# AlexeyAB/yolo2_light

Measured on NVIDIA H100. Metric: images/sec, higher is better.
Workload: dtype bf16

## Files before the change

### yolo2_light_b200/api.py

```python
from __future__ import annotations

import ctypes as C
import os
from typing import List, Optional

import numpy as np

_HERE = os.path.dirname(os.path.abspath(__file__))
LIB_PATH = os.environ.get("YB_LIB") or os.path.join(_HERE, "libyolo2_light_b200.so")

YB_CONVOLUTIONAL, YB_MAXPOOL, YB_SOFTMAX, YB_ROUTE, YB_SHORTCUT = 0, 3, 4, 8, 13
YB_REGION, YB_YOLO, YB_UPSAMPLE, YB_REORG, YB_BLANK = 21, 22, 23, 24, 25
YB_LOGISTIC, YB_RELU, YB_LINEAR, YB_LEAKY = 0, 1, 3, 7
YB_PREC_BF16_TC, YB_PREC_FP32 = 0, 1
YB_QUANT_NONE, YB_QUANT_CPU, YB_QUANT_GPU = 0, 1, 2
LAYER_NAMES = {0: "CONVOLUTIONAL", 3: "MAXPOOL", 4: "SOFTMAX", 8: "ROUTE", 13: "SHORTCUT", 21: "REGION", 22: "YOLO",
               23: "UPSAMPLE", 24: "REORG", 25: "BLANK"}


class YbError(RuntimeError):
    pass


class LayerDesc(C.Structure):
# ... 107 lines not shown
    return L


EXPORTED_SYMBOLS = [
    "yb_set_abort_on_error", "yb_last_error", "yb_version", "yb_parse_network_cfg", "yb_load_weights_upto",
    "yb_fuse_conv_batchnorm", "yb_calculate_binary_weights", "yb_quantinization_and_get_multipliers",
    "yb_network_from_layers", "yb_free_network", "yb_network_num_layers", "yb_network_dims", "yb_network_layer",
    "yb_network_layer_outputs", "yb_network_input_calibration", "yb_set_batch_network", "yb_network_set_device",
    "yb_network_set_precision", "yb_network_set_option", "yb_network_get_info", "yb_network_tc_plan", "yb_network_detect", "yb_network_calibrate", "yb_entropy_calibration",
    "yb_network_input_histogram", "yb_map_evaluate", "yb_network_predict", "yb_network_predict_quantized",
    "yb_network_predict_cudnn_quantized",
    "yb_network_predict_image_u8", "yb_network_fetch_input", "yb_network_submit", "yb_network_collect", "yb_network_layer_output", "yb_network_forward_device", "yb_network_sync_outputs", "yb_network_fetch_layer",
    "yb_network_fetch_counts", "yb_forward_convolutional_layer", "yb_network_weight_arena",
    "yb_network_last_launches", "yb_network_profile", "yb_op_kind_name", "yb_network_op_kernels", "yb_get_network_boxes", "yb_alloc_pinned",
    "yb_free_pinned", "yb_network_submit_u8", "yb_network_collect_detections", "yb_network_set_devices",
    "yb_network_predict_batch", "yb_network_batch_output", "yb_network_replication", "yb_network_predict_frames_u8",
    "yb_network_detect_frames", "yb_network_submit_frames_u8", "yb_network_predict_device_frames",
    "yb_network_submit_device_frames", "yb_network_set_letterbox",
]


TC_PLAN_FIELDS = ("kernel", "kind", "TW", "TH", "BN", "BK", "nt", "bstat", "stages", "sps", "grid", "num_work", "tma_epi",
                  "jshift", "out_ldc")
TC_PLAN_KERNELS = ("k_conv_tc", "k_conv_tc_reg", "k_stem_tc", "k_stem_s2_tc")
TC_PLAN_KINDS = ("bf16", "s8", "xnor", "tf32", "s8_gpu")


def _check(ok: bool):
    if not ok:
        raise YbError(lib().yb_last_error().decode(errors="replace"))


def _np(ptr, count, dtype):
    if not ptr or count <= 0:
        return None
    return np.ctypeslib.as_array(ptr, shape=(count,)).view(dtype)


class Network:

    def __init__(self, handle: int):
        self._h = C.c_void_p(handle)
        self._refresh()

    def _refresh(self):
        d = (C.c_int * 8)()
        lib().yb_network_dims(self._h, d)
# ... 509 lines not shown
```

### yolo2_light_b200/csrc/yb_conv_tc.cu

```cuda
#include <cuda.h>
#include <cuda_bf16.h>
#include <cuda_runtime.h>

#include <algorithm>
#include <climits>
#include <cstdlib>
#include <cstring>
#include <memory>
#include <string>
#include <type_traits>
#include <vector>

#include "yb_conv_tc.cuh"
#include "yb_cuda.h"

namespace yb {

namespace {

constexpr int TC_BM = 128;
constexpr int TC_EPI_WARPS = 8;
constexpr int TC_THREADS = 32 * TC_EPI_WARPS + 32;
constexpr int TC_PRODUCER_WARP = TC_EPI_WARPS;
constexpr int TC_ACC_BAR = 3;
// ... 24 lines not shown
    int yolo_per;
    int PR, row_off;
    int OH, OW, OHp, OWp;
    int size, cblocks, kblocks;
    int BK, BN;
    int stride2;
    int xoff, yoff;
    int stages;
    uint32_t stage_bytes, a_bytes, b_bytes;
    int bstat;
    uint32_t bstat_bytes;
    int tma_epi;
    uint32_t stg_bytes;
    int acc_pitch;
    int pool_fmt, jshift;
    float pool_mult;
    signed char *pool_out; long pool_ldc; int pool_Hp, pool_Wp;
    int sps;
    TcSmem sm;
    uint32_t desc_hi;
    char *out; long out_ldc; int n;
    const char *res;
    const float *bias; int act, act2;
    unsigned long long *stats;
    int dbg;
};

__device__ __forceinline__ uint32_t smem_u32(const void *p) { return (uint32_t)__cvta_generic_to_shared(p); }

__device__ __forceinline__ bool elect_one() {
    uint32_t pred = 0;
    asm volatile(
        "{\n\t.reg .b32 rx;\n\t.reg .pred px;\n\telect.sync rx|px, %1;\n\t@px mov.s32 %0, 1;\n\t}"
        : "+r"(pred) : "r"(0xffffffffu));
    return pred != 0;
}

__device__ __forceinline__ void mbar_init(uint32_t bar, uint32_t count) {
    asm volatile("mbarrier.init.shared::cta.b64 [%0], %1;" ::"r"(bar), "r"(count));
}
__device__ __forceinline__ void mbar_arrive_expect_tx(uint32_t bar, uint32_t bytes) {
    asm volatile("mbarrier.arrive.expect_tx.shared::cta.b64 _, [%0], %1;" ::"r"(bar), "r"(bytes) : "memory");
}
__device__ __forceinline__ void mbar_arrive(uint32_t bar) {
    asm volatile("mbarrier.arrive.shared::cta.b64 _, [%0];" ::"r"(bar) : "memory");
}
// ... 10 lines not shown
    while (!mbar_try_wait(bar, parity))
        if (clock64() - t0 > 4000000000LL) __trap();
}

__device__ __forceinline__ void tma_load_3d(uint32_t dst, const CUtensorMap *tm, uint32_t bar, int c0, int c1, int c2) {
    asm volatile(
        "cp.async.bulk.tensor.3d.shared::cluster.global.tile.mbarrier::complete_tx::bytes [%0], [%1, {%3, %4, %5}], [%2];"
        ::"r"(dst), "l"(tm), "r"(bar), "r"(c0), "r"(c1), "r"(c2) : "memory");
}
__device__ __forceinline__ uint64_t l2_policy_evict_first() {
    uint64_t pol;
    asm volatile("createpolicy.fractional.L2::evict_first.b64 %0, 1.0;" : "=l"(pol));
    return pol;
}
__device__ __forceinline__ void tma_load_3d_hint(uint32_t dst, const CUtensorMap *tm, uint32_t bar, int c0, int c1, int c2, uint64_t pol) {
    asm volatile(
        "cp.async.bulk.tensor.3d.shared::cluster.global.tile.mbarrier::complete_tx::bytes.L2::cache_hint [%0], [%1, {%3, %4, %5}], [%2], %6;"
        ::"r"(dst), "l"(tm), "r"(bar), "r"(c0), "r"(c1), "r"(c2), "l"(pol) : "memory");
}
__device__ __forceinline__ void tma_load_2d(uint32_t dst, const CUtensorMap *tm, uint32_t bar, int c0, int c1) {
    asm volatile(
        "cp.async.bulk.tensor.2d.shared::cluster.global.tile.mbarrier::complete_tx::bytes [%0], [%1, {%3, %4}], [%2];"
        ::"r"(dst), "l"(tm), "r"(bar), "r"(c0), "r"(c1) : "memory");
}
__device__ __forceinline__ void tma_load_5d(uint32_t dst, const CUtensorMap *tm, uint32_t bar, int c0, int c1, int c2,
                                            int c3, int c4) {
    asm volatile(
        "cp.async.bulk.tensor.5d.shared::cluster.global.tile.mbarrier::complete_tx::bytes [%0], [%1, {%3, %4, %5, %6, %7}], [%2];"
        ::"r"(dst), "l"(tm), "r"(bar), "r"(c0), "r"(c1), "r"(c2), "r"(c3), "r"(c4) : "memory");
}

__device__ __forceinline__ void tma_store_3d(const CUtensorMap *tm, uint32_t src, int c0, int c1, int c2) {
    asm volatile("cp.async.bulk.tensor.3d.global.shared::cta.bulk_group [%0, {%2, %3, %4}], [%1];"
                 ::"l"(tm), "r"(src), "r"(c0), "r"(c1), "r"(c2) : "memory");
}
__device__ __forceinline__ void tma_store_commit() { asm volatile("cp.async.bulk.commit_group;" ::: "memory"); }
__device__ __forceinline__ void tma_store_wait_read0() { asm volatile("cp.async.bulk.wait_group.read 0;" ::: "memory"); }
__device__ __forceinline__ void tma_store_wait_all() { asm volatile("cp.async.bulk.wait_group 0;" ::: "memory"); }
__device__ __forceinline__ void named_bar_sync(int id, int nthreads) {
    asm volatile("bar.sync %0, %1;" ::"r"(id), "r"(nthreads) : "memory");
}
__device__ __forceinline__ void prefetch_tmap(const CUtensorMap *tm) { asm volatile("prefetch.tensormap [%0];" ::"l"(tm) : "memory"); }
__device__ __forceinline__ void fence_mbar_init() { asm volatile("fence.mbarrier_init.release.cluster;" ::: "memory"); }
__device__ __forceinline__ void pdl_wait_and_launch() {
    asm volatile("griddepcontrol.wait;" ::: "memory");
    asm volatile("griddepcontrol.launch_dependents;" ::: "memory");
// ... 893 lines not shown
                const unsigned long long dst = optr[px];
                if (dst)
                    *reinterpret_cast<uint4 *>(dst + (unsigned long long)(part * 16)) =
                        *reinterpret_cast<const uint4 *>(a_tile + px * 64 + ((part ^ ((px >> 1) & 3)) << 4));
            }
        } else if (ok) {
#pragma unroll
            for (int g = 0; g < 4; ++g) {
                if (g * 8 >= p.nf) break;
                float r[8];
#pragma unroll
                for (int j = 0; j < 8; ++j) {
                    const float a = __uint_as_float(acc[g * 8 + j]) + bias_s[g * 8 + j];
                    r[j] = (p.act == ACT_LEAKY) ? fmaxf(a, 0.1f * a) : a;
                }
                reinterpret_cast<uint4 *>(orow)[g] = make_uint4(pack_bf16x2(r[0], r[1]), pack_bf16x2(r[2], r[3]),
                                                                pack_bf16x2(r[4], r[5]), pack_bf16x2(r[6], r[7]));
            }
        }
        __syncthreads();
    }
}

constexpr int S2_TW = 16, S2_TH = 8;
constexpr int S2_RW = 2 * S2_TW + 1, S2_RH = 2 * S2_TH + 1;
constexpr int S2_ROWS = 640;
constexpr uint32_t S2_B1 = 0;
constexpr uint32_t S2_BS = 9u * 4096u;
constexpr uint32_t S2_U = S2_BS + 2048u;
constexpr uint32_t S2_SETS_KX = 17u * 1024u;
constexpr uint32_t S2_STG = (uint32_t)S2_ROWS * 64u;
constexpr uint32_t S2_MISC = S2_U + S2_STG + 2u * 8192u;
constexpr int S2_PH = S2_RH + 2, S2_PW = S2_RW + 2, S2_PP = 36;
constexpr size_t S2_SMEM = 1024 + S2_MISC + 4 * (32 + 64 + 256) + 4 * 3 * S2_PH * S2_PP;
static_assert(S2_STG + 2u * 8192u >= 3u * S2_SETS_KX, "sets must fit the shared region");

template <bool U8>
__global__ void __launch_bounds__(256, 2) k_stem_s2_tc(StemTcP p) {
    extern __shared__ uint8_t smem_raw[];
    uint8_t *sm = smem_raw + ((1024u - (smem_u32(smem_raw) & 1023u)) & 1023u);
    const uint32_t base = smem_u32(sm), U = base + S2_U;
    float *bias0_s = reinterpret_cast<float *>(sm + S2_MISC), *bias1_s = bias0_s + 32, *lut = bias1_s + 64, *patch = lut + 256;
    const int t = threadIdx.x, lane = t & 31;
    const int warp = __shfl_sync(0xffffffffu, t >> 5, 0), wg = warp >> 2;
    if constexpr (U8) lut[t] = (float)((double)(float)t / 255.0);
    if (t < 32) bias0_s[t] = p.bias[t];
// ... 91 lines not shown
                Wg<TC_BF16, 32>::mma(ds[c], wg_desc(U + (uint32_t)(5 * wg + c) * 4096u + 32u * k, hi), wg_desc(base + S2_BS + 32u * k, hi), (uint32_t)k);
        wg_commit();
        wg_wait<0>();
#pragma unroll
        for (int c = 0; c < 5; ++c) wg_fence_operand(ds[c]);
        __syncthreads();

        {
#pragma unroll
            for (int c = 0; c < 5; ++c)
#pragma unroll
                for (int h = 0; h < 2; ++h) {
                    const int i = 64 * (5 * wg + c) + rl + 8 * h;
                    if (i >= S2_RW * S2_RH) continue;
                    const int sy = i / S2_RW, sx = i - sy * S2_RW, y = gy0 + sy, x = gx0 + sx;
                    const bool in_img = y >= 0 && y < p.H && x >= 0 && x < p.W;
                    uint32_t v[4];
#pragma unroll
                    for (int j = 0; j < 4; ++j) {
                        float a = ds[c][4 * j + 2 * h] + bias0_s[8 * j + cq], b = ds[c][4 * j + 2 * h + 1] + bias0_s[8 * j + cq + 1];
                        if (leaky0) { a = fmaxf(a, 0.1f * a); b = fmaxf(b, 0.1f * b); }
                        v[j] = in_img ? pack_bf16x2(a, b) : 0u;
                    }
                    const uint32_t set = U + ((sy & 1) ? 9u * 1024u : 0u) + (uint32_t)(sy >> 1) * 1024u + 2u * (uint32_t)cq;
                    auto put = [&](int kx, int ox) {
                        const uint32_t row = set + (uint32_t)kx * S2_SETS_KX + (uint32_t)ox * 64u;
#pragma unroll
                        for (int j = 0; j < 4; ++j)
                            asm volatile("st.shared.b32 [%0], %1;" ::"r"(row + ((uint32_t)(j ^ ((ox >> 1) & 3)) << 4)), "r"(v[j]));
                    };
                    const bool odd = sx & 1, last = sx == 2 * S2_TW;
                    put(odd ? 1 : last ? 2 : 0, last ? (sx >> 1) - 1 : sx >> 1);
                    if (!odd && !last && sx >= 2) put(2, (sx >> 1) - 1);
                }
        }
        asm volatile("fence.proxy.async.shared::cta;" ::: "memory");
        __syncthreads();

        if (tile + (int)gridDim.x < p.ntiles) load_patch(tile + gridDim.x, pv);

        float d[32];
#pragma unroll
        for (int i = 0; i < 32; ++i) d[i] = 0.f;
        wg_fence_operand(d);
        wg_fence();
#pragma unroll
        for (int r = 0; r < 9; ++r) {
            const int ky = r / 3, kx = r % 3;
            const uint32_t a = U + (uint32_t)kx * S2_SETS_KX + ((ky & 1) ? 9u * 1024u : 0u) + (uint32_t)(ky >> 1) * 1024u + (uint32_t)wg * 4096u;
            const uint32_t b = base + S2_B1 + (uint32_t)r * 4096u;
#pragma unroll
            for (int k = 0; k < 2; ++k)
                Wg<TC_BF16, 64>::mma(d, wg_desc(a + 32u * k, hi), wg_desc(b + 32u * k, hi), (r > 0 || k > 0) ? 1u : 0u);
        }
        wg_commit();
        wg_wait<0>();
        wg_fence_operand(d);
        __syncthreads();

        const uint32_t stg = U + S2_STG + (uint32_t)wg * 8192u;
        float b1[16];
#pragma unroll
        for (int j = 0; j < 8; ++j) { b1[2 * j] = bias1_s[8 * j + cq]; b1[2 * j + 1] = bias1_s[8 * j + cq + 1]; }
#pragma unroll
        for (int h = 0; h < 2; ++h) {
            const int q = rl + 8 * h;
#pragma unroll
            for (int j = 0; j < 8; ++j) {
                float a = d[4 * j + 2 * h] + b1[2 * j], b = d[4 * j + 2 * h + 1] + b1[2 * j + 1];
                if (leaky1) { a = fmaxf(a, 0.1f * a); b = fmaxf(b, 0.1f * b); }
                asm volatile("st.shared.b32 [%0], %1;" ::"r"(stg + (uint32_t)q * 128u + ((uint32_t)(j ^ (q & 7)) << 4) + 2u * (uint32_t)cq),
                             "r"(pack_bf16x2(a, b)) : "memory");
            }
        }
        if (wg == 0) named_bar_sync(1, 128);
        else named_bar_sync(2, 128);
#pragma unroll
        for (int k = 0; k < 4; ++k) {
            const int idx = (t & 127) + 128 * k, q = idx >> 3, ch = idx & 7;
            const int oy = oy0 + 4 * wg + (q >> 4), ox = ox0 + (q & 15);
            if (oy < p.OH && ox < p.OW) {
                uint4 o;
                asm volatile("ld.shared.v4.b32 {%0, %1, %2, %3}, [%4];" : "=r"(o.x), "=r"(o.y), "=r"(o.z), "=r"(o.w)
                             : "r"(stg + (uint32_t)q * 128u + ((uint32_t)(ch ^ (q & 7)) << 4)) : "memory");
                *reinterpret_cast<uint4 *>(p.out + ((size_t)(n * p.OHp + oy + 1) * p.OWp + ox + 1) * (size_t)p.out_ldc * 2 + ch * 16) = o;
            }
        }
    }
}

typedef CUresult (*EncodeTiledFn)(CUtensorMap *, CUtensorMapDataType, cuuint32_t, void *, const cuuint64_t *,
                                  const cuuint64_t *, const cuuint32_t *, const cuuint32_t *, CUtensorMapInterleave,
                                  CUtensorMapSwizzle, CUtensorMapL2promotion, CUtensorMapFloatOOBfill);

EncodeTiledFn encode_fn() {
    static EncodeTiledFn fn = nullptr;
    if (!fn) {
        void *p = nullptr;
        cudaDriverEntryPointQueryResult q;
        if (cudaGetDriverEntryPoint("cuTensorMapEncodeTiled", &p, cudaEnableDefault, &q) != cudaSuccess || !p)
            fatal_throw("cuTensorMapEncodeTiled not available from the driver");
        fn = reinterpret_cast<EncodeTiledFn>(p);
    }
    return fn;
}

}

using TcKernel = void (*)(CUtensorMap, CUtensorMap, CUtensorMap, CUtensorMap, CUtensorMap, TcParams);

struct TcPlan {
    CUtensorMap tmA, tmB, tmO, tmO1, tmR;
    TcParams p;
    TcKernel kernel;
    bool reg;
    int grid;
    size_t smem;
    char desc[96];
    DevBuf<unsigned long long> stats;
};

namespace {

int sm_count() {
    int dev = 0, sms = 132;
    cudaGetDevice(&dev);
    cudaDeviceGetAttribute(&sms, cudaDevAttrMultiProcessorCount, dev);
    return sms;
}

bool is_integer(int kind) { return kind == TC_S8 || kind == TC_S8_GPU || kind == TC_XNOR; }
int elem_size(int kind) { return kind == TC_TF32 ? 4 : is_integer(kind) ? 1 : 2; }
int operand_channels(const TcConv &c) { return is_integer(c.kind) ? c.in.ldc : c.l->c; }

bool geometry_ok(const Layer &l) {
    if (l.stride == 1) return (l.size == 3 && l.pad == 1) || (l.size == 1 && l.pad == 0);
    return l.stride == 2 && l.size == 3 && l.pad == 1 && l.h % 2 == 0 && l.w % 2 == 0;
}
// ... 229 lines not shown
    plan_tiles(p, c, reg, sms);
    plan_epilogue(p, c, reg);
    plan_ring(p, reg);
    plan->smem = tc_smem_layout(p, reg);
    p.dbg = c.sw.dbg;
    snprintf(plan->desc, sizeof(plan->desc), "%dx%dx%d -> n%d k%d s%d%s", l.c, l.h, l.w, l.n, l.size, l.stride, reg ? " reg" : "");
    encode_maps(*plan, c, reg);
    plan->grid = std::min(p.num_work, grid_cap(sms, c.sw.grid));
    const bool st = c.sw.stats;
    plan->reg = reg;
    if (reg) plan->kernel = st ? k_conv_tc_reg<true> : k_conv_tc_reg<false>;
    else if (is_integer(c.kind)) plan->kernel = st ? k_conv_tc<true, 2> : k_conv_tc<false, 2>;
    else plan->kernel = st ? k_conv_tc<true, 0> : k_conv_tc<false, 0>;
    if (cudaFuncSetAttribute((const void *)plan->kernel, cudaFuncAttributeMaxDynamicSharedMemorySize, 227 * 1024) != cudaSuccess)
        fatal_throw("cudaFuncSetAttribute(k_conv_tc) failed");
    if (st) {
        plan->stats.ensure(TC_NSTATS * (size_t)plan->grid);
        p.stats = plan->stats.get();
        cudaMemset(p.stats, 0, sizeof(unsigned long long) * TC_NSTATS * plan->grid);
    }
    return plan;
}

struct StemPlan { StemTcP p; int grid; bool s2; };
int tc_stem_supported(const Layer &l, const TV &out) {
    return l.c == 3 && l.size == 3 && l.stride == 1 && l.pad == 1 && (l.n == 16 || l.n == 32) &&
           (l.activation == YB_LEAKY || l.activation == YB_LINEAR) && out.base && out.ldc % 8 == 0 &&
           (reinterpret_cast<uintptr_t>(out.base) & 15) == 0;
}
StemPlanPtr tc_stem_make_plan(const Layer &l, const TV &out, const void *d_w, const float *d_bias) {
    StemPlanPtr sp(new StemPlan());
    StemTcP &p = sp->p;
    p.out = out.base; p.out_ldc = out.ldc; p.w = reinterpret_cast<const __nv_bfloat16 *>(d_w); p.bias = d_bias;
    p.N = out.N; p.H = l.h; p.W = l.w; p.OHp = out.Hp; p.OWp = out.Wp; p.nf = l.n; p.act = l.activation;
    p.npix = (long)out.N * l.h * l.w;
    if (p.npix >= (1L << 31) - 256) fatal_throw("stem plan: more than 2^31 pixels per batch");
    p.ntiles = (int)((p.npix + 127) / 128);
    sp->grid = std::min(p.ntiles, sm_count() * 8);
    return sp;
}
int tc_stem_s2_supported(const Layer &l0, const Layer &l1, const TV &out1) {
    return l0.n == 32 && l1.c == 32 && l1.n == 64 && l1.size == 3 && l1.stride == 2 && l1.pad == 1 && l1.h == l0.h && l1.w == l0.w &&
           l0.h % 2 == 0 && l0.w % 2 == 0 && (l1.activation == YB_LEAKY || l1.activation == YB_LINEAR) && out1.base && out1.P == 1 &&
           out1.H == l0.h / 2 && out1.W == l0.w / 2 && out1.ldc % 8 == 0 && (reinterpret_cast<uintptr_t>(out1.base) & 15) == 0;
}
StemPlanPtr tc_stem_s2_make_plan(const Layer &l0, const Layer &l1, const TV &out1, const void *d_w, const float *d_bias,
// ... 20 lines not shown
void tc_stem_launch(const StemPlan &sp, const float *d_in_nchw, cudaStream_t s) {
    StemTcP p = sp.p;
    p.in = d_in_nchw;
    if (sp.s2) k_stem_s2_tc<false><<<sp.grid, 256, S2_SMEM, s>>>(p);
    else k_stem_tc<false><<<sp.grid, 128, 0, s>>>(p);
}
void tc_stem_launch_u8(const StemPlan &sp, const unsigned char *d_in_hwc, cudaStream_t s) {
    StemTcP p = sp.p;
    p.in8 = d_in_hwc;
    if (sp.s2) k_stem_s2_tc<true><<<sp.grid, 256, S2_SMEM, s>>>(p);
    else k_stem_tc<true><<<sp.grid, 128, 0, s>>>(p);
}

namespace {
int copy_fields(const int (&f)[TC_PLAN_NFIELDS], int *fields, int n) {
    const int k = std::max(0, std::min(n, (int)TC_PLAN_NFIELDS));
    for (int i = 0; i < k; ++i) fields[i] = f[i];
    return k;
}
}

int tc_plan_fields(const TcPlan &plan, int *fields, int n) {
    const TcParams &p = plan.p;
    const int f[TC_PLAN_NFIELDS] = {plan.reg ? TC_PLAN_CONV_REG : TC_PLAN_CONV, p.kind, p.TW, p.TH, p.BN, p.BK,
                                    p.nt, p.bstat, p.stages, p.sps, plan.grid, p.num_work, p.tma_epi, p.jshift,
                                    p.out ? (int)p.out_ldc : 0};
    return copy_fields(f, fields, n);
}

int tc_stem_plan_fields(const StemPlan &sp, int *fields, int n) {
    const int f[TC_PLAN_NFIELDS] = {sp.s2 ? TC_PLAN_STEM_S2 : TC_PLAN_STEM, TC_BF16, sp.s2 ? S2_TW : -1, sp.s2 ? S2_TH : -1,
                                    sp.s2 ? 64 : -1, -1, -1, -1, -1, -1, sp.grid, sp.p.ntiles, -1, -1, (int)sp.p.out_ldc};
    return copy_fields(f, fields, n);
}

void tc_launch(const TcPlan &P, cudaStream_t s) {
    cudaLaunchConfig_t cfg{};
    cfg.gridDim = dim3((unsigned)P.grid); cfg.blockDim = dim3((unsigned)(P.reg ? TCR_THREADS : TC_THREADS));
    cfg.dynamicSmemBytes = P.smem; cfg.stream = s;
    cudaLaunchAttribute attr[1];
    attr[0].id = cudaLaunchAttributeProgrammaticStreamSerialization;
    attr[0].val.programmaticStreamSerializationAllowed = 1;
    cfg.attrs = attr; cfg.numAttrs = 1;
    cudaLaunchKernelEx(&cfg, P.kernel, P.tmA, P.tmB, P.tmO, P.tmO1, P.tmR, P.p);
}

void TcPlanDelete::operator()(TcPlan *plan) const {
    if (plan->p.stats) {
        std::vector<unsigned long long> h(TC_NSTATS * (size_t)plan->grid);
        cudaDeviceSynchronize();
        cudaMemcpy(h.data(), plan->p.stats, h.size() * sizeof(unsigned long long), cudaMemcpyDeviceToHost);
        double m[TC_NSTATS] = {0};
        for (int b = 0; b < plan->grid; ++b) for (int k = 0; k < TC_NSTATS; ++k) m[k] += (double)h[TC_NSTATS * b + k] / plan->grid;
        fprintf(stderr, "TCSTATS %-28s tiles/cta %.1f kb %d sps %d BN %d | producer: wait_empty %.0f tma_issue %.0f total %.0f | ",
                plan->desc, (double)plan->p.num_work / plan->grid, plan->p.kblocks, plan->p.sps, plan->p.BN,
                m[STAT_PROD_WAIT_EMPTY], m[STAT_PROD_TMA_ISSUE], m[STAT_PROD_TOTAL]);
        if (plan->reg)
            fprintf(stderr, "consumers: wait_full %.0f wait_ready %.0f (first item %.0f) total %.0f | store: wait_full %.0f wait_read %.0f\n",
                    m[STAT_CONS_WAIT_FULL], m[STAT_CONS_WAIT_READY], m[STAT_CONS_FIRST_READY], m[STAT_CONS_TOTAL],
                    m[STAT_STORE_WAIT_FULL], m[STAT_STORE_WAIT_READ]);
        else fprintf(stderr, "consumers: wait_full %.0f total %.0f\n", m[STAT_CONS_WAIT_FULL], m[STAT_CONS_TOTAL]);
// ... 7 lines not shown
```

### yolo2_light_b200/csrc/yb_conv_tc.cuh

```cuda
#pragma once
#include <cuda_runtime.h>

#include <memory>

#include "yb_device.cuh"
#include "yb_model.h"

namespace yb {

struct TcSwitches {
    int bn = 0;
    int grid = 0;
    bool no_bstat = false;
    bool stats = false;
    int dbg = 0;
};

struct TcConv {
    TcKind kind = TC_BF16;
    const Layer *l = nullptr;
    TV in{};
    TV out{};
    bool out_bf16 = false;
    TV res{};
// ... 4 lines not shown
    float alpha1 = 0.f;
    const float *mean = nullptr;
    int *acc_out = nullptr;
    float *yolo_out = nullptr;
    int yolo_classes = 0;
    SideFmt pool_fmt = SIDE_NONE;
    float pool_mult = 0.f;
    TV pool_next{};
    TcSwitches sw{};
};

struct TcPlan;
struct StemPlan;
struct TcPlanDelete {
    void operator()(TcPlan *plan) const;
    void operator()(StemPlan *plan) const;
};
using TcPlanPtr = std::unique_ptr<TcPlan, TcPlanDelete>;
using StemPlanPtr = std::unique_ptr<StemPlan, TcPlanDelete>;

int tc_conv_supported(const TcConv &c);
TcPlanPtr tc_make_plan(const TcConv &c);
void tc_launch(const TcPlan &plan, cudaStream_t s);

int tc_stem_supported(const Layer &l, const TV &out);
StemPlanPtr tc_stem_make_plan(const Layer &l, const TV &out, const void *d_w_32x32_bf16, const float *d_bias);
int tc_stem_s2_supported(const Layer &l0, const Layer &l1, const TV &out1);
StemPlanPtr tc_stem_s2_make_plan(const Layer &l0, const Layer &l1, const TV &out1, const void *d_w_32x32_bf16,
                                 const float *d_bias, const void *d_w1_bf16, const float *d_bias1, int max_grid);
void tc_stem_launch(const StemPlan &plan, const float *d_in_nchw, cudaStream_t s);
void tc_stem_launch_u8(const StemPlan &plan, const unsigned char *d_in_hwc, cudaStream_t s);

enum { TC_PLAN_CONV = 0, TC_PLAN_CONV_REG = 1, TC_PLAN_STEM = 2, TC_PLAN_STEM_S2 = 3, TC_PLAN_NFIELDS = 15 };
int tc_plan_fields(const TcPlan &plan, int *fields, int n);
int tc_stem_plan_fields(const StemPlan &plan, int *fields, int n);

}
```

### yolo2_light_b200/csrc/yb_engine.cu

```cuda
#include "yb_engine.h"

#include <cuda_bf16.h>
#include <cuda_runtime.h>
#include <dlfcn.h>

#include <algorithm>
#include <cmath>
#include <cstdlib>
#include <cstring>

#include "yb_conv_tc.cuh"
#include "yb_cuda.h"
#include "yb_kernels.cuh"
#include "yb_detect.cuh"

namespace yb {

const char *op_kind_name(int k) {
    static const char *names[] = {"input", "conv_simt", "conv_tc", "binarize", "conv_xnor", "quantize",
                                  "conv_int8", "maxpool", "upsample", "shortcut", "route_copy", "reorg",
                                  "yolo", "region", "conv_tc_i8", "conv_tc_tf32"};
    return (k >= 0 && k < 16) ? names[k] : "?";
}

// ... 1 lines not shown
static inline size_t dt_size(int dt) { return dt == DT_F32 ? 4 : dt == DT_BF16 ? 2 : dt == DT_S8 ? 1 : 4; }
#define BY_DT(k, dt) ((dt) == DT_F32 ? k<float> : k<__nv_bfloat16>)

struct Op {
    int kind;
    int layer;
    std::function<void(const float *, cudaStream_t)> launch;
    std::function<void(const unsigned char *, cudaStream_t)> launch_u8;
    const void *kernel = nullptr;
};

struct ConvWeights {
    size_t w_f32 = (size_t)-1, w_bf16 = (size_t)-1, w_s8 = (size_t)-1, w_bits = (size_t)-1;
    size_t w_f32km = (size_t)-1;
    size_t bias = (size_t)-1, mean = (size_t)-1;
    int ldw = 0;
    int ldn = 0;
    int cpad = 0;
};

struct Switches {
    bool no_graph, no_nccl, no_tc, no_tf32, no_stem, no_stem_tc, no_stem_u8, no_stem_pool_fuse, no_stem_s2_fuse,
         no_conv_pool_fuse, no_pool_fuse, no_yolo_fuse;
    bool no_fuse;
    bool xnor_tc;
    int xnor_tc_minc;
    TcSwitches tc;
    static Switches read() {
        auto set = [](const char *name) { return getenv(name) != nullptr; };
        auto num = [](const char *name) { const char *v = getenv(name); return v ? atoi(v) : 0; };
        const char *xtc = getenv("YB_XNOR_TC"), *minc = getenv("YB_XNOR_TC_MINC"), *nf = getenv("YB_NO_FUSE");
        return Switches{set("YB_NO_GRAPH"), set("YB_NO_NCCL"), set("YB_NO_TC"), set("YB_NO_TF32"), set("YB_NO_STEM"),
                        set("YB_NO_STEM_TC"), set("YB_NO_STEM_U8"), set("YB_NO_STEM_POOL_FUSE"), set("YB_NO_STEM_S2_FUSE"),
                        set("YB_NO_CONV_POOL_FUSE"), set("YB_NO_POOL_FUSE"), set("YB_NO_YOLO_FUSE"),
                        nf && nf[0] == '1', !(xtc && xtc[0] == '0'), minc ? atoi(minc) : 16,
                        TcSwitches{set("YB_TC_BN") ? std::max(num("YB_TC_BN"), 1) : 0, num("YB_TC_GRID"), set("YB_TC_NO_BSTAT"),
                                   set("YB_TC_STATS"), num("YB_TC_DBG")}};
    }
};

struct Engine {
    EngineOptions opt;
    Switches sw{};
    int batch = 0;
    int act_dt = DT_F32;
    Stream stream;
    DevBuf<char> act_arena, w_arena;
    DevBuf<float> d_input;
    std::vector<TV> out_tv;
    std::vector<int> out_dt;
    struct Final { DevBuf<float> d; PinnedBuf<float> h; };
    std::vector<Final> finals;
    std::vector<DevBuf<int32_t>> counts;
    std::vector<Op> ops;
    TV in0{};
    int in0_dt = DT_F32;
    GraphExec graph_exec;
// ... 64 lines not shown
            if (l.type == YB_SHORTCUT) cons[l.index].push_back(i);
        }
    }
    return cons;
}

template <typename T> struct same_type { using type = T; };


enum FirstOp { FIRST_NHWC, FIRST_STEM_SIMT, FIRST_STEM_TC, FIRST_STEM_S2, FIRST_STEM_POOL };
enum ConvPath { CP_NONE, CP_TC, CP_TF32, CP_SIMT, CP_XNOR_FALLBACK, CP_XNOR_TC, CP_XNOR_SMALLK, CP_XNOR_GENERAL, CP_I8_TC, CP_I8_SIMT };

struct LayerPlan {
    int variant = 0;
    int path = CP_NONE;
    int fused_into = -1;
    bool fused_sc = false;
    bool yolo_fused = false;
    SideFmt pool = SIDE_NONE;
    bool pool_in_conv = false;
    bool pool_to_side = false;
    bool prefilled = false;
    bool in_first_op = false;
    int out_dt = DT_F32;
    SideFmt side = SIDE_NONE;
    int side_ld = 0;
    bool has_out = false;
    bool materialised = false;
    int owner = -1, coff = 0;
    int ldc = 0;
};

static char *const kLayoutBase = reinterpret_cast<char *>(uintptr_t(1) << 40);

template <typename F>
static void for_each_weight(const Layer &l, F &&put) {
    const int taps = l.size * l.size;
    for (int f = 0; f < l.n; ++f)
        for (int c = 0; c < l.c; ++c)
            for (int t = 0; t < taps; ++t) put(f, c, t, ((size_t)f * l.c + c) * taps + t);
}

template <int NF>
static StemW<NF> stem_weights(const Layer &l0) {
    StemW<NF> w{};
    for_each_weight(l0, [&](int f, int c, int t, size_t k) { w.w[(t * 3 + c) * NF + f] = l0.weights[k]; });
// ... 303 lines not shown
    }

    void plan_fusions() {
        for (int i = 0; i < nl; ++i) {
            LayerPlan &p = L[i];
            if (!is_conv(i) || p.in_first_op) continue;
            const SideFmt pf = conv_pool_fmt(i);
            bool pool = false;
            if (p.path == CP_XNOR_TC || p.path == CP_I8_TC) {
                pool = pf != SIDE_NONE && tc_conv_supported(tc_conv(i, false, pf));
            } else if (p.path == CP_XNOR_SMALLK) {
                pool = pf == SIDE_PM1_S8 || pf == SIDE_BITS;
            }
            if (pool) {
                p.pool = pf;
                L[i + 1].pool_in_conv = L[i + 2].prefilled = true;
                p.materialised = L[i + 1].materialised = false;
            }
            if ((p.path == CP_TF32 || p.path == CP_TC) && opt.fuse && p.fused_into < 0 && p.out_dt == DT_F32 && i + 1 < nl &&
                layer(i + 1).type == YB_YOLO && sole_reader(i, i + 1) && !sw.no_yolo_fuse) {
                p.yolo_fused = L[i + 1].yolo_fused = true;
                p.materialised = false;
            }
        }
        for (int i = 0; i + 1 < nl; ++i) {
            if (layer(i).type != YB_MAXPOOL || L[i].in_first_op || L[i].pool_in_conv) continue;
            const Layer &c = layer(i + 1);
            if (opt.fuse && in_dt(i) == DT_F32 && sole_reader(i, i + 1) && c.type == YB_CONVOLUTIONAL && L[i + 1].variant != 0 &&
                L[i + 1].side != SIDE_NONE && !xnor_fallback(c) && !sw.no_pool_fuse) {
                L[i].pool_to_side = L[i + 1].prefilled = true;
                L[i].materialised = false;
            }
        }
    }

    void place() {
        size_t total = 0;
        auto take = [&](size_t bytes) { const size_t off = total; total += align_up(bytes, 1024); return off; };
        const size_t in0_off = first == FIRST_NHWC ? take(tv_bytes(B, net.h, net.w, net.c, P, ADT)) : 0;
        for (int i = 0; i < nl; ++i) {
            const Layer &l = layer(i);
            if (L[i].materialised && !is_alias(i) && L[i].owner < 0)
                buf_off[i] = take(tv_bytes(B, l.out_h, l.out_w, L[i].ldc, P, L[i].out_dt));
        }
        for (int i = 0; i < nl; ++i) {
            const Layer &l = layer(i);
// ... 144 lines not shown
            const bool bf16 = L[0].out_dt == DT_BF16;
            const unsigned grid = (unsigned)(((long)B * H * W + 127) / 128);
            if (l0.n == 32)
                push_input_kernel(OP_CONV_SIMT, 0, bf16 ? k_conv_stem<32, __nv_bfloat16> : k_conv_stem<32, float, true>, grid, 128,
                                  e.out_tv[0], stem_weights<32>(l0), act, H, W);
            else
                push_input_kernel(OP_CONV_SIMT, 0, bf16 ? k_conv_stem<16, __nv_bfloat16> : k_conv_stem<16, float, true>, grid, 128,
                                  e.out_tv[0], stem_weights<16>(l0), act, H, W);
        } else {
            push_input_kernel(OP_INPUT, -1, BY_DT(k_input_nchw_to_nhwc, ADT), grid_for((long)e.in0.N * e.in0.H * e.in0.W), 256, e.in0);
        }
    }

    void push_int_input(int kind, int i, int j, const TV &tin, int size, int stride, int pad) {
        const SideFmt f = L[j].side;
        void (*const k[4])(TV, TV, int, int, int, float) = {k_int_input<SIDE_S8>, k_int_input<SIDE_PM1_S8>, k_int_input<SIDE_BITS>,
                                                            k_int_input<SIDE_S8_SAT>};
        const TV q = side_placed(j);
        push_kernel(kind, i, k[f - SIDE_S8], grid_for((long)B * q.H * q.W * int_input_groups(f, tin.C)), 256, 0, tin, q, size, stride, pad,
                    side_mult(j));
    }

    void emit_conv(int i) {
        const TV tin = i == 0 ? e.in0 : e.out_tv[i - 1];
        const SideFmt f = L[i].side;
        if (!L[i].prefilled && side_int(f))
            push_int_input(side_s8(f) ? OP_QUANTIZE : OP_BINARIZE, i, i, tin, 1, 1, 0);
        if (L[i].variant == 0) emit_conv_fp32(i, tin);
        else if (L[i].variant == 1) emit_conv_xnor(i, tin);
        else emit_conv_int8(i);
    }

    void push_conv_simt(int kind, int i, void (*k)(SimtP), const TV &tin, const TV &tout, const TV &res = TV{}, int act2 = ACT_LINEAR) {
        const Layer &l = layer(i);
        const LayerPlan &p = L[i];
        const int taps = l.size * l.size;
        const long M = (long)B * l.out_h * l.out_w;
        SimtP sp{};
        sp.in = tin; sp.out = tout; sp.res = res;
        sp.bias = bias(i);
        sp.n = l.n; sp.size = l.size; sp.stride = l.stride; sp.pad = l.pad;
        sp.act = l.activation; sp.act2 = act2; sp.M = M;
        if (p.side == SIDE_BITS) {
            sp.CW = p.side_ld;
            sp.w = e.w_arena.get() + cw[i].w_bits;
            sp.mean = reinterpret_cast<const float *>(e.w_arena.get() + cw[i].mean);
// ... 730 lines not shown
```

Baseline: 3183.

## Fuse 1x1+3x3 residual block into a single tensor-core kernel

Adds k_res_block_tc, which computes a 64->32 1x1 conv, a 32->64 3x3 conv and the residual add in one kernel. The 1x1 intermediate and the residual tile stay in shared memory instead of round-tripping through global memory. The planner enables it for matching bf16 conv pairs, by default only when the activation exceeds L2 size and the preceding layer belongs to the first op. It also factors the shared set_put/sets_conv3x3/stage_flush helpers out of the stem kernel. The kernel recomputes the 1x1 over the halo and syncs per tile without pipelining, which may cost throughput.

```diff
diff --git a/yolo2_light_b200/api.py b/yolo2_light_b200/api.py
--- a/yolo2_light_b200/api.py
+++ b/yolo2_light_b200/api.py
@@ -153,7 +153,7 @@
 
 TC_PLAN_FIELDS = ("kernel", "kind", "TW", "TH", "BN", "BK", "nt", "bstat", "stages", "sps", "grid", "num_work", "tma_epi",
                   "jshift", "out_ldc")
-TC_PLAN_KERNELS = ("k_conv_tc", "k_conv_tc_reg", "k_stem_tc", "k_stem_s2_tc")
+TC_PLAN_KERNELS = ("k_conv_tc", "k_conv_tc_reg", "k_stem_tc", "k_stem_s2_tc", "k_res_block_tc")
 TC_PLAN_KINDS = ("bf16", "s8", "xnor", "tf32", "s8_gpu")
 
 
diff --git a/yolo2_light_b200/csrc/yb_conv_tc.cu b/yolo2_light_b200/csrc/yb_conv_tc.cu
--- a/yolo2_light_b200/csrc/yb_conv_tc.cu
+++ b/yolo2_light_b200/csrc/yb_conv_tc.cu
@@ -70,6 +70,7 @@
     char *out; long out_ldc; int n;
     const char *res;
     const float *bias; int act, act2;
+    const __nv_bfloat16 *w1, *w3; const float *bias1; int act1;
     unsigned long long *stats;
     int dbg;
 };
@@ -126,6 +127,11 @@
     asm volatile(
         "cp.async.bulk.tensor.2d.shared::cluster.global.tile.mbarrier::complete_tx::bytes [%0], [%1, {%3, %4}], [%2];"
         ::"r"(dst), "l"(tm), "r"(bar), "r"(c0), "r"(c1) : "memory");
+}
+__device__ __forceinline__ void tma_load_4d(uint32_t dst, const CUtensorMap *tm, uint32_t bar, int c0, int c1, int c2, int c3) {
+    asm volatile(
+        "cp.async.bulk.tensor.4d.shared::cluster.global.tile.mbarrier::complete_tx::bytes [%0], [%1, {%3, %4, %5, %6}], [%2];"
+        ::"r"(dst), "l"(tm), "r"(bar), "r"(c0), "r"(c1), "r"(c2), "r"(c3) : "memory");
 }
 __device__ __forceinline__ void tma_load_5d(uint32_t dst, const CUtensorMap *tm, uint32_t bar, int c0, int c1, int c2,
                                             int c3, int c4) {
@@ -1065,6 +1071,47 @@
     }
 }
 
+
+__device__ __forceinline__ void set_put(uint32_t set, int ox, int cq, const uint32_t (&v)[4]) {
+    const uint32_t row = set + (uint32_t)ox * 64u + 2u * (uint32_t)cq;
+#pragma unroll
+    for (int j = 0; j < 4; ++j) asm volatile("st.shared.b32 [%0], %1;" ::"r"(row + ((uint32_t)(j ^ ((ox >> 1) & 3)) << 4)), "r"(v[j]));
+}
+template <typename F>
+__device__ __forceinline__ void sets_conv3x3(float (&d)[32], F &&tap_a, uint32_t b) {
+    const uint32_t hi = ((8u * 64u) >> 4) | (2u << 30);
+#pragma unroll
+    for (int i = 0; i < 32; ++i) d[i] = 0.f;
+    wg_fence_operand(d);
+    wg_fence();
+#pragma unroll
+    for (int r = 0; r < 9; ++r) {
+        const uint32_t a = tap_a(r / 3, r % 3);
+#pragma unroll
+        for (int k = 0; k < 2; ++k)
+            Wg<TC_BF16, 64>::mma(d, wg_desc(a + 32u * k, hi), wg_desc(b + (uint32_t)r * 4096u + 32u * k, hi), (r > 0 || k > 0) ? 1u : 0u);
+    }
+    wg_commit();
+    wg_wait<0>();
+    wg_fence_operand(d);
+}
+__device__ __forceinline__ void stage_put(uint32_t stg, int q, int j, int cq, uint32_t v) {
+    asm volatile("st.shared.b32 [%0], %1;" ::"r"(stg + (uint32_t)q * 128u + ((uint32_t)(j ^ (q & 7)) << 4) + 2u * (uint32_t)cq), "r"(v) : "memory");
+}
+template <typename F>
+__device__ __forceinline__ void stage_flush(uint32_t stg, int t, F &&dst) {
+#pragma unroll
+    for (int k = 0; k < 4; ++k) {
+        const int idx = (t & 127) + 128 * k, q = idx >> 3, ch = idx & 7;
+        if (char *o = dst(q)) {
+            uint4 v;
+            asm volatile("ld.shared.v4.b32 {%0, %1, %2, %3}, [%4];" : "=r"(v.x), "=r"(v.y), "=r"(v.z), "=r"(v.w)
+                         : "r"(stg + (uint32_t)q * 128u + ((uint32_t)(ch ^ (q & 7)) << 4)) : "memory");
+            *reinterpret_cast<uint4 *>(o + ch * 16) = v;
+        }
+    }
+}
+
 constexpr int S2_TW = 16, S2_TH = 8;
 constexpr int S2_RW = 2 * S2_TW + 1, S2_RH = 2 * S2_TH + 1;
 constexpr int S2_ROWS = 640;
@@ -1202,13 +1249,8 @@
                         if (leaky0) { a = fmaxf(a, 0.1f * a); b = fmaxf(b, 0.1f * b); }
                         v[j] = in_img ? pack_bf16x2(a, b) : 0u;
                     }
-                    const uint32_t set = U + ((sy & 1) ? 9u * 1024u : 0u) + (uint32_t)(sy >> 1) * 1024u + 2u * (uint32_t)cq;
-                    auto put = [&](int kx, int ox) {
-                        const uint32_t row = set + (uint32_t)kx * S2_SETS_KX + (uint32_t)ox * 64u;
-#pragma unroll
-                        for (int j = 0; j < 4; ++j)
-                            asm volatile("st.shared.b32 [%0], %1;" ::"r"(row + ((uint32_t)(j ^ ((ox >> 1) & 3)) << 4)), "r"(v[j]));
-                    };
+                    const uint32_t set = U + ((sy & 1) ? 9u * 1024u : 0u) + (uint32_t)(sy >> 1) * 1024u;
+                    auto put = [&](int kx, int ox) { set_put(set + (uint32_t)kx * S2_SETS_KX, ox, cq, v); };
                     const bool odd = sx & 1, last = sx == 2 * S2_TW;
                     put(odd ? 1 : last ? 2 : 0, last ? (sx >> 1) - 1 : sx >> 1);
                     if (!odd && !last && sx >= 2) put(2, (sx >> 1) - 1);
@@ -1220,22 +1262,9 @@
         if (tile + (int)gridDim.x < p.ntiles) load_patch(tile + gridDim.x, pv);
 
         float d[32];
-#pragma unroll
-        for (int i = 0; i < 32; ++i) d[i] = 0.f;
-        wg_fence_operand(d);
-        wg_fence();
-#pragma unroll
-        for (int r = 0; r < 9; ++r) {
-            const int ky = r / 3, kx = r % 3;
-            const uint32_t a = U + (uint32_t)kx * S2_SETS_KX + ((ky & 1) ? 9u * 1024u : 0u) + (uint32_t)(ky >> 1) * 1024u + (uint32_t)wg * 4096u;
-            const uint32_t b = base + S2_B1 + (uint32_t)r * 4096u;
-#pragma unroll
-            for (int k = 0; k < 2; ++k)
-                Wg<TC_BF16, 64>::mma(d, wg_desc(a + 32u * k, hi), wg_desc(b + 32u * k, hi), (r > 0 || k > 0) ? 1u : 0u);
-        }
-        wg_commit();
-        wg_wait<0>();
-        wg_fence_operand(d);
+        sets_conv3x3(d, [&](int ky, int kx) {
+            return U + (uint32_t)kx * S2_SETS_KX + ((ky & 1) ? 9u * 1024u : 0u) + (uint32_t)(ky >> 1) * 1024u + (uint32_t)wg * 4096u;
+        }, base + S2_B1);
         __syncthreads();
 
         const uint32_t stg = U + S2_STG + (uint32_t)wg * 8192u;
@@ -1249,23 +1278,154 @@
             for (int j = 0; j < 8; ++j) {
                 float a = d[4 * j + 2 * h] + b1[2 * j], b = d[4 * j + 2 * h + 1] + b1[2 * j + 1];
                 if (leaky1) { a = fmaxf(a, 0.1f * a); b = fmaxf(b, 0.1f * b); }
-                asm volatile("st.shared.b32 [%0], %1;" ::"r"(stg + (uint32_t)q * 128u + ((uint32_t)(j ^ (q & 7)) << 4) + 2u * (uint32_t)cq),
-                             "r"(pack_bf16x2(a, b)) : "memory");
+                stage_put(stg, q, j, cq, pack_bf16x2(a, b));
             }
         }
         if (wg == 0) named_bar_sync(1, 128);
         else named_bar_sync(2, 128);
+        stage_flush(stg, t, [&](int q) -> char * {
+            const int oy = oy0 + 4 * wg + (q >> 4), ox = ox0 + (q & 15);
+            return oy < p.OH && ox < p.OW ? p.out + ((size_t)(n * p.OHp + oy + 1) * p.OWp + ox + 1) * (size_t)p.out_ldc * 2 : nullptr;
+        });
+    }
+}
+
+constexpr int RB_BW = S2_TW + 2, RB_BH = S2_TH + 2;
+constexpr uint32_t RB_XBYTES = (uint32_t)(RB_BW * RB_BH) * 128u;
+constexpr uint32_t RB_X = 0;
+constexpr uint32_t RB_R = 192u * 128u;
+constexpr uint32_t RB_W1 = RB_R + 128u * 128u;
+constexpr uint32_t RB_W3 = RB_W1 + 32u * 128u;
+constexpr uint32_t RB_SETS = RB_W3 + 9u * 4096u;
+constexpr uint32_t RB_SETS_KX = (uint32_t)RB_BH * 1024u;
+constexpr uint32_t RB_MISC = RB_SETS + 3u * RB_SETS_KX;
+constexpr size_t RB_SMEM = 1024 + RB_MISC + 4 * (32 + 64) + 8;
+static_assert(3u * RB_SETS_KX >= 2u * 8192u, "the staging tiles must fit the sets");
+static_assert(RB_XBYTES <= RB_R, "x box");
+
+__global__ void __launch_bounds__(256, 2)
+k_res_block_tc(const __grid_constant__ CUtensorMap tmX, const __grid_constant__ CUtensorMap, const __grid_constant__ CUtensorMap,
+               const __grid_constant__ CUtensorMap, const __grid_constant__ CUtensorMap, const TcParams p) {
+    extern __shared__ uint8_t smem_raw[];
+    const uint32_t base = smem_base(smem_raw), X = base + RB_X, R = base + RB_R, SETS = base + RB_SETS, bar = base + RB_MISC + 4u * 96u;
+    float *bias1_s = reinterpret_cast<float *>(smem_ptr(base + RB_MISC)), *bias_s = bias1_s + 32;
+    const int t = threadIdx.x, lane = t & 31;
+    const int warp = __shfl_sync(0xffffffffu, t >> 5, 0), wg = warp >> 2;
+    if (t == 0) {
+        prefetch_tmap(&tmX);
+        mbar_init(bar, 1);
+        fence_mbar_init();
+    }
+    if (t < 32) bias1_s[t] = p.bias1[t];
+    if (t < 64) bias_s[t] = p.bias[t];
+    {
+        const int f = t >> 3, j = t & 7;
+        *reinterpret_cast<uint4 *>(smem_ptr(base + RB_W1 + f * 128 + ((j ^ (f & 7)) << 4))) = *reinterpret_cast<const uint4 *>(p.w1 + f * 64 + j * 8);
+    }
+    for (int i = t; i < 9 * 64 * 4; i += 256) {
+        const int r = i >> 8, f = (i >> 2) & 63, j = i & 3;
+        *reinterpret_cast<uint4 *>(smem_ptr(base + RB_W3 + r * 4096 + f * 64 + ((j ^ ((f >> 1) & 3)) << 4))) =
+            *reinterpret_cast<const uint4 *>(p.w3 + f * 288 + r * 32 + j * 8);
+    }
+    asm volatile("fence.proxy.async.shared::cta;" ::: "memory");
+    __syncthreads();
+    pdl_wait_and_launch();
+
+    const int yt = p.jt;
+    auto load_x = [&](int tile) {
+        const int tx = tile % p.xt, rest = tile / p.xt, ty = rest % yt, n = rest / yt;
+        mbar_arrive_expect_tx(bar, RB_XBYTES);
+        tma_load_4d(X, &tmX, bar, 0, tx * S2_TW, ty * S2_TH, n);
+    };
+    if (t == 0 && (int)blockIdx.x < p.num_work) load_x(blockIdx.x);
+
+    const uint32_t hi128 = ((8u * 128u) >> 4) | (1u << 30);
+    const bool leaky1 = p.act1 == ACT_LEAKY, leaky = p.act == ACT_LEAKY, leaky2 = p.act2 == ACT_LEAKY;
+    const int rl = 16 * (warp & 3) + (lane >> 2), cq = 2 * (lane & 3);
+    uint32_t phase = 0;
+    for (int tile = blockIdx.x; tile < p.num_work; tile += gridDim.x, phase ^= 1u) {
+        const int tx = tile % p.xt, rest = tile / p.xt, ty = rest % yt, n = rest / yt;
+        const int ox0 = tx * S2_TW, oy0 = ty * S2_TH;
+        mbar_wait(bar, phase);
+
+        float ds[2][16];
+#pragma unroll
+        for (int c = 0; c < 2; ++c)
+#pragma unroll
+            for (int i = 0; i < 16; ++i) ds[c][i] = 0.f;
+#pragma unroll
+        for (int c = 0; c < 2; ++c) wg_fence_operand(ds[c]);
+        wg_fence();
+#pragma unroll
+        for (int c = 0; c < 2; ++c)
+#pragma unroll
+            for (int k = 0; k < 4; ++k)
+                Wg<TC_BF16, 32>::mma(ds[c], wg_desc(X + (uint32_t)(2 * wg + c) * 8192u + 32u * k, hi128), wg_desc(base + RB_W1 + 32u * k, hi128),
+                                     k > 0 ? 1u : 0u);
+        wg_commit();
+        wg_wait<0>();
+#pragma unroll
+        for (int c = 0; c < 2; ++c) wg_fence_operand(ds[c]);
+        __syncthreads();
 #pragma unroll
         for (int k = 0; k < 4; ++k) {
-            const int idx = (t & 127) + 128 * k, q = idx >> 3, ch = idx & 7;
+            const int idx = t + 256 * k, q = idx >> 3, j = idx & 7, rb = ((q >> 4) + 1) * RB_BW + (q & 15) + 1;
+            uint4 v;
+            asm volatile("ld.shared.v4.b32 {%0, %1, %2, %3}, [%4];" : "=r"(v.x), "=r"(v.y), "=r"(v.z), "=r"(v.w)
+                         : "r"(X + (uint32_t)rb * 128u + ((uint32_t)(j ^ (rb & 7)) << 4)) : "memory");
+            asm volatile("st.shared.v4.b32 [%0], {%1, %2, %3, %4};" ::"r"(R + (uint32_t)q * 128u + ((uint32_t)(j ^ (q & 7)) << 4)),
+                         "r"(v.x), "r"(v.y), "r"(v.z), "r"(v.w) : "memory");
+        }
+
+#pragma unroll
+        for (int c = 0; c < 2; ++c)
+#pragma unroll
+            for (int h = 0; h < 2; ++h) {
+                const int i = 64 * (2 * wg + c) + rl + 8 * h;
+                if (i >= RB_BW * RB_BH) continue;
+                const int hy = i / RB_BW, hx = i - hy * RB_BW, y = oy0 - 1 + hy, x = ox0 - 1 + hx;
+                const bool in_img = y >= 0 && y < p.OH && x >= 0 && x < p.OW;
+                uint32_t v[4];
+#pragma unroll
+                for (int j = 0; j < 4; ++j) {
+                    float a = ds[c][4 * j + 2 * h] + bias1_s[8 * j + cq], b = ds[c][4 * j + 2 * h + 1] + bias1_s[8 * j + cq + 1];
+                    if (leaky1) { a = fmaxf(a, 0.1f * a); b = fmaxf(b, 0.1f * b); }
+                    v[j] = in_img ? pack_bf16x2(a, b) : 0u;
+                }
+#pragma unroll
+                for (int kx = 0; kx < 3; ++kx)
+                    if (hx - kx >= 0 && hx - kx < S2_TW) set_put(SETS + (uint32_t)kx * RB_SETS_KX + (uint32_t)hy * 1024u, hx - kx, cq, v);
+            }
+        asm volatile("fence.proxy.async.shared::cta;" ::: "memory");
+        __syncthreads();
+        if (t == 0 && tile + (int)gridDim.x < p.num_work) load_x(tile + gridDim.x);
+
+        float d[32];
+        sets_conv3x3(d, [&](int ky, int kx) { return SETS + (uint32_t)kx * RB_SETS_KX + (uint32_t)(ky + 4 * wg) * 1024u; }, base + RB_W3);
+        __syncthreads();
+
+        const uint32_t stg = SETS + (uint32_t)wg * 8192u;
+#pragma unroll
+        for (int h = 0; h < 2; ++h) {
+            const int q = rl + 8 * h;
+            const int qr = 64 * wg + q;
+#pragma unroll
+            for (int j = 0; j < 8; ++j) {
+                uint32_t u;
+                asm volatile("ld.shared.b32 %0, [%1];" : "=r"(u) : "r"(R + (uint32_t)qr * 128u + ((uint32_t)(j ^ (qr & 7)) << 4) + 2u * (uint32_t)cq));
+                float a = d[4 * j + 2 * h] + bias_s[8 * j + cq], b = d[4 * j + 2 * h + 1] + bias_s[8 * j + cq + 1];
+                if (leaky) { a = fmaxf(a, 0.1f * a); b = fmaxf(b, 0.1f * b); }
+                a += __uint_as_float(u << 16);
+                b += __uint_as_float(u & 0xffff0000u);
+                if (leaky2) { a = fmaxf(a, 0.1f * a); b = fmaxf(b, 0.1f * b); }
+                stage_put(stg, q, j, cq, pack_bf16x2(a, b));
+            }
+        }
+        __syncthreads();
+        stage_flush(stg, t, [&](int q) -> char * {
             const int oy = oy0 + 4 * wg + (q >> 4), ox = ox0 + (q & 15);
-            if (oy < p.OH && ox < p.OW) {
-                uint4 o;
-                asm volatile("ld.shared.v4.b32 {%0, %1, %2, %3}, [%4];" : "=r"(o.x), "=r"(o.y), "=r"(o.z), "=r"(o.w)
-                             : "r"(stg + (uint32_t)q * 128u + ((uint32_t)(ch ^ (q & 7)) << 4)) : "memory");
-                *reinterpret_cast<uint4 *>(p.out + ((size_t)(n * p.OHp + oy + 1) * p.OWp + ox + 1) * (size_t)p.out_ldc * 2 + ch * 16) = o;
-            }
-        }
+            return oy < p.OH && ox < p.OW ? p.out + ((size_t)(n * p.OHp + oy + 1) * p.OWp + ox + 1) * (size_t)p.out_ldc * 2 : nullptr;
+        });
     }
 }
 
@@ -1294,6 +1454,7 @@
     TcParams p;
     TcKernel kernel;
     bool reg;
+    bool res_block = false;
     int grid;
     size_t smem;
     char desc[96];
@@ -1569,6 +1730,59 @@
     return plan;
 }
 
+int tc_res_block_supported(const TcConv &c1, const TcConv &c3) {
+    const Layer &l1 = *c1.l, &l3 = *c3.l;
+    auto act_ok = [](int a) { return a == YB_LEAKY || a == YB_LINEAR; };
+    auto aligned = [](const TV &t) { return t.base && t.P == 1 && (reinterpret_cast<uintptr_t>(t.base) & 15) == 0; };
+    return c1.kind == TC_BF16 && c3.kind == TC_BF16 && c3.out_bf16 && l1.c == 64 && l1.n == 32 && l1.size == 1 && l1.stride == 1 &&
+           l1.pad == 0 && l3.c == 32 && l3.n == 64 && l3.size == 3 && l3.stride == 1 && l3.pad == 1 && l3.h == l1.h && l3.w == l1.w &&
+           act_ok(l1.activation) && act_ok(l3.activation) && act_ok(c3.act2) && aligned(c1.in) && c1.in.ldc == 64 && c1.in.C == 64 &&
+           c3.res.base == c1.in.base && c3.res.ldc == c1.in.ldc && aligned(c3.out) && c3.out.ldc % 8 == 0 && c3.out.H == l1.h &&
+           c3.out.W == l1.w && c1.in.H == l1.h && c1.in.W == l1.w && !c1.yolo_out && !c3.yolo_out && c1.pool_fmt == SIDE_NONE &&
+           c3.pool_fmt == SIDE_NONE;
+}
+
+TcPlanPtr tc_res_block_make_plan(const TcConv &c1, const TcConv &c3) {
+    if (!tc_res_block_supported(c1, c3)) fatal_throw("tc plan: residual block not supported by k_res_block_tc");
+    const Layer &l1 = *c1.l;
+    const TV &x = c1.in, &y = c3.out;
+    TcPlanPtr plan(new TcPlan());
+    plan->res_block = true;
+    TcParams &p = plan->p;
+    p.kind = TC_BF16; p.TW = S2_TW; p.TH = S2_TH; p.BN = 64; p.BK = -1; p.nt = -1; p.bstat = -1; p.stages = -1; p.sps = -1;
+    p.tma_epi = -1; p.jshift = -1;
+    p.N = x.N; p.OH = l1.h; p.OW = l1.w; p.OHp = y.Hp; p.OWp = y.Wp;
+    p.xt = (p.OW + S2_TW - 1) / S2_TW; p.jt = (p.OH + S2_TH - 1) / S2_TH;
+    const long ntiles = (long)p.N * p.xt * p.jt;
+    if (ntiles >= INT_MAX) fatal_throw("tc plan: too many tiles");
+    p.num_work = (int)ntiles;
+    p.out = y.base; p.out_ldc = y.ldc; p.n = 64;
+    p.res = x.base;
+    p.w1 = reinterpret_cast<const __nv_bfloat16 *>(c1.w); p.bias1 = c1.bias; p.act1 = l1.activation;
+    p.w3 = reinterpret_cast<const __nv_bfloat16 *>(c3.w); p.bias = c3.bias; p.act = c3.l->activation; p.act2 = c3.act2;
+    {
+        cuuint64_t dims[4] = {64, (cuuint64_t)x.Wp, (cuuint64_t)x.Hp, (cuuint64_t)x.N};
+        cuuint64_t strides[3] = {(cuuint64_t)x.ldc * 2, (cuuint64_t)x.Wp * x.ldc * 2, (cuuint64_t)x.Hp * x.Wp * x.ldc * 2};
+        cuuint32_t box[4] = {64, (cuuint32_t)RB_BW, (cuuint32_t)RB_BH, 1};
+        cuuint32_t es[4] = {1, 1, 1, 1};
+        const CUresult r = encode_fn()(&plan->tmA, CU_TENSOR_MAP_DATA_TYPE_BFLOAT16, 4, x.base, dims, strides, box, es,
+                                       CU_TENSOR_MAP_INTERLEAVE_NONE, CU_TENSOR_MAP_SWIZZLE_128B, CU_TENSOR_MAP_L2_PROMOTION_L2_128B,
+                                       CU_TENSOR_MAP_FLOAT_OOB_FILL_NONE);
+        if (r != CUDA_SUCCESS) fatal_throw("cuTensorMapEncodeTiled(x box) failed: " + std::to_string((int)r));
+    }
+    plan->tmB = plan->tmO = plan->tmO1 = plan->tmR = plan->tmA;
+    plan->kernel = k_res_block_tc;
+    plan->smem = RB_SMEM;
+    plan->grid = std::min(p.num_work, grid_cap(2 * sm_count(), c3.sw.grid));
+    snprintf(plan->desc, sizeof(plan->desc), "res block 64x%dx%d", l1.h, l1.w);
+    if (cudaFuncSetAttribute((const void *)k_res_block_tc, cudaFuncAttributeMaxDynamicSharedMemorySize, (int)RB_SMEM) != cudaSuccess ||
+        cudaFuncSetAttribute((const void *)k_res_block_tc, cudaFuncAttributePreferredSharedMemoryCarveout, 100) != cudaSuccess)
+        fatal_throw("cudaFuncSetAttribute(k_res_block_tc) failed");
+    return plan;
+}
+
+const void *tc_plan_kernel(const TcPlan &plan) { return (const void *)plan.kernel; }
+
 struct StemPlan { StemTcP p; int grid; bool s2; };
 int tc_stem_supported(const Layer &l, const TV &out) {
     return l.c == 3 && l.size == 3 && l.stride == 1 && l.pad == 1 && (l.n == 16 || l.n == 32) &&
@@ -1635,7 +1849,7 @@
 
 int tc_plan_fields(const TcPlan &plan, int *fields, int n) {
     const TcParams &p = plan.p;
-    const int f[TC_PLAN_NFIELDS] = {plan.reg ? TC_PLAN_CONV_REG : TC_PLAN_CONV, p.kind, p.TW, p.TH, p.BN, p.BK,
+    const int f[TC_PLAN_NFIELDS] = {plan.res_block ? TC_PLAN_RES_BLOCK : plan.reg ? TC_PLAN_CONV_REG : TC_PLAN_CONV, p.kind, p.TW, p.TH, p.BN, p.BK,
                                     p.nt, p.bstat, p.stages, p.sps, plan.grid, p.num_work, p.tma_epi, p.jshift,
                                     p.out ? (int)p.out_ldc : 0};
     return copy_fields(f, fields, n);
@@ -1649,7 +1863,7 @@
 
 void tc_launch(const TcPlan &P, cudaStream_t s) {
     cudaLaunchConfig_t cfg{};
-    cfg.gridDim = dim3((unsigned)P.grid); cfg.blockDim = dim3((unsigned)(P.reg ? TCR_THREADS : TC_THREADS));
+    cfg.gridDim = dim3((unsigned)P.grid); cfg.blockDim = dim3((unsigned)(P.res_block ? 256 : P.reg ? TCR_THREADS : TC_THREADS));
     cfg.dynamicSmemBytes = P.smem; cfg.stream = s;
     cudaLaunchAttribute attr[1];
     attr[0].id = cudaLaunchAttributeProgrammaticStreamSerialization;
diff --git a/yolo2_light_b200/csrc/yb_conv_tc.cuh b/yolo2_light_b200/csrc/yb_conv_tc.cuh
--- a/yolo2_light_b200/csrc/yb_conv_tc.cuh
+++ b/yolo2_light_b200/csrc/yb_conv_tc.cuh
@@ -50,6 +50,10 @@
 int tc_conv_supported(const TcConv &c);
 TcPlanPtr tc_make_plan(const TcConv &c);
 void tc_launch(const TcPlan &plan, cudaStream_t s);
+const void *tc_plan_kernel(const TcPlan &plan);
+
+int tc_res_block_supported(const TcConv &c1, const TcConv &c3);
+TcPlanPtr tc_res_block_make_plan(const TcConv &c1, const TcConv &c3);
 
 int tc_stem_supported(const Layer &l, const TV &out);
 StemPlanPtr tc_stem_make_plan(const Layer &l, const TV &out, const void *d_w_32x32_bf16, const float *d_bias);
@@ -59,7 +63,7 @@
 void tc_stem_launch(const StemPlan &plan, const float *d_in_nchw, cudaStream_t s);
 void tc_stem_launch_u8(const StemPlan &plan, const unsigned char *d_in_hwc, cudaStream_t s);
 
-enum { TC_PLAN_CONV = 0, TC_PLAN_CONV_REG = 1, TC_PLAN_STEM = 2, TC_PLAN_STEM_S2 = 3, TC_PLAN_NFIELDS = 15 };
+enum { TC_PLAN_CONV = 0, TC_PLAN_CONV_REG = 1, TC_PLAN_STEM = 2, TC_PLAN_STEM_S2 = 3, TC_PLAN_RES_BLOCK = 4, TC_PLAN_NFIELDS = 15 };
 int tc_plan_fields(const TcPlan &plan, int *fields, int n);
 int tc_stem_plan_fields(const StemPlan &plan, int *fields, int n);
 
diff --git a/yolo2_light_b200/csrc/yb_engine.cu b/yolo2_light_b200/csrc/yb_engine.cu
--- a/yolo2_light_b200/csrc/yb_engine.cu
+++ b/yolo2_light_b200/csrc/yb_engine.cu
@@ -47,6 +47,7 @@
 struct Switches {
     bool no_graph, no_nccl, no_tc, no_tf32, no_stem, no_stem_tc, no_stem_u8, no_stem_pool_fuse, no_stem_s2_fuse,
          no_conv_pool_fuse, no_pool_fuse, no_yolo_fuse;
+    int res_block_fuse;
     bool no_fuse;
     bool xnor_tc;
     int xnor_tc_minc;
@@ -58,6 +59,7 @@
         return Switches{set("YB_NO_GRAPH"), set("YB_NO_NCCL"), set("YB_NO_TC"), set("YB_NO_TF32"), set("YB_NO_STEM"),
                         set("YB_NO_STEM_TC"), set("YB_NO_STEM_U8"), set("YB_NO_STEM_POOL_FUSE"), set("YB_NO_STEM_S2_FUSE"),
                         set("YB_NO_CONV_POOL_FUSE"), set("YB_NO_POOL_FUSE"), set("YB_NO_YOLO_FUSE"),
+                        getenv("YB_RES_BLOCK_FUSE") ? num("YB_RES_BLOCK_FUSE") : -1,
                         nf && nf[0] == '1', !(xtc && xtc[0] == '0'), minc ? atoi(minc) : 16,
                         TcSwitches{set("YB_TC_BN") ? std::max(num("YB_TC_BN"), 1) : 0, num("YB_TC_GRID"), set("YB_TC_NO_BSTAT"),
                                    set("YB_TC_STATS"), num("YB_TC_DBG")}};
@@ -168,6 +170,7 @@
     bool pool_to_side = false;
     bool prefilled = false;
     bool in_first_op = false;
+    bool res_block = false;
     int out_dt = DT_F32;
     SideFmt side = SIDE_NONE;
     int side_ld = 0;
@@ -517,6 +520,21 @@
                 p.yolo_fused = L[i + 1].yolo_fused = true;
                 p.materialised = false;
             }
+        }
+        int l2 = 0;
+        CUDA_OK(cudaDeviceGetAttribute(&l2, cudaDevAttrL2CacheSize, opt.device));
+        for (int i = 1; i + 2 < nl; ++i) {
+            if (!opt.fuse || sw.res_block_fuse == 0) break;
+            if (sw.res_block_fuse < 0 && (!L[i - 1].in_first_op || tv_bytes(B, layer(i).h, layer(i).w, 64, P, DT_BF16) <= (size_t)l2))
+                continue;
+            if (!is_conv(i) || !is_conv(i + 1) || L[i].in_first_op || L[i + 1].in_first_op || L[i + 1].fused_into != i + 2) continue;
+            if (layer(i + 2).index != i - 1 || !sole_reader(i, i + 1)) continue;
+            if (L[i].variant != 0 || L[i + 1].variant != 0 || L[i].path != CP_TC || L[i + 1].path != CP_TC || ADT != DT_BF16 ||
+                in_dt(i) != DT_BF16 || L[i].out_dt != DT_BF16 || L[i].fused_into >= 0 || L[i].yolo_fused || L[i].pool != SIDE_NONE)
+                continue;
+            if (!tc_res_block_supported(tc_conv(i, false, SIDE_NONE), tc_conv(i + 1, false, SIDE_NONE))) continue;
+            L[i].res_block = true;
+            L[i].materialised = false;
         }
         for (int i = 0; i + 1 < nl; ++i) {
             if (layer(i).type != YB_MAXPOOL || L[i].in_first_op || L[i].pool_in_conv) continue;
@@ -707,6 +725,14 @@
     }
 
     void emit_conv(int i) {
+        if (L[i].res_block) return;
+        if (i > 0 && L[i - 1].res_block) {
+            e.tc_plans.emplace_back(i, tc_res_block_make_plan(tc_conv(i - 1, true, SIDE_NONE), tc_conv(i, true, SIDE_NONE)));
+            const TcPlan *plan = e.tc_plans.back().second.get();
+            e.n_tc += 2;
+            push(OP_CONV_TC, i, [plan](const float *, cudaStream_t s) { tc_launch(*plan, s); }, tc_plan_kernel(*plan));
+            return;
+        }
         const TV tin = i == 0 ? e.in0 : e.out_tv[i - 1];
         const SideFmt f = L[i].side;
         if (!L[i].prefilled && side_int(f))
```

New measurement: 3228, median of 6. 1.01x the previous value.
